# zm0612/funny_lidar_slam

Hardware: NVIDIA H100
Metric: scans/sec (higher is better)
Workload: dtype f64

## Files before the change

### funny_lidar_slam_b200/csrc/fls_api.cu

```cuda
#include <algorithm>
#include <cmath>
#include <cstdlib>
#include <cstring>
#include <new>
#include <vector>

#include "fls_frontend.h"
#include "fls_gn.cuh"
#include "fls_handle.h"

namespace fls {

static thread_local std::string g_last_error;
void set_last_error(const std::string& s) { g_last_error = s; }
const char* last_error_cstr() { return g_last_error.c_str(); }

Handle::Handle(const fls_config& c) : cfg(c) {
    try {
        init();
    } catch (...) {
        release();
        throw;
    }
}
// ... 117 lines not shown
        st->h2d_bytes = h2d_bytes;
        st->d2h_bytes = d2h_bytes;
    }
}

void Handle::set_fit_cloud(const float4* d, size_t n) {
    fit_cloud.reserve(n);
    if (n) FLS_CUDA(cudaMemcpyAsync(fit_cloud.p, d, n * sizeof(float4), cudaMemcpyDeviceToDevice, stream));
    set_fit_view(fit_cloud.p, n);
}

void Handle::set_fit_view(const float4* d, size_t n) {
    fit_pts = d;
    fit_cloud_n = n;
    fit_cloud_version++;
}

GnParams Handle::gn_params(int method, int min_effective) const {
    GnParams p;
    p.method = method;
    p.max_iterations = cfg.max_iterations;
    p.min_effective = min_effective;
    p.rot_thres = cfg.rotation_converge_thres;
    p.pos_thres = cfg.position_converge_thres;
    return p;
}

unsigned Handle::next_ll_epoch(size_t n_records) {
    const size_t cap0 = ll_rows.cap;
    ll_rows.reserve(n_records);
    if (ll_rows.cap != cap0) FLS_CUDA(cudaMemsetAsync(ll_rows.p, 0, ll_rows.cap * sizeof(uint4), stream));
    match_epoch = (match_epoch + 1) & 0xffffffu;
    if (match_epoch == 0) match_epoch = 1;
    return match_epoch << 8;
}

unsigned char* Handle::batch_table(size_t bytes) {
    if (bytes > h_batch_cap) {
        if (h_batch) cudaFreeHost(h_batch);
        h_batch = nullptr;
        h_batch_cap = 0;
        FLS_CUDA(cudaMallocHost(&h_batch, bytes * 2));
        h_batch_cap = bytes * 2;
    }
    d_batch.reserve(bytes);
    return h_batch;
}

void Handle::send_batch_table(size_t bytes) {
    FLS_CUDA(cudaMemcpyAsync(d_batch.p, h_batch, bytes, cudaMemcpyHostToDevice, stream));
    h2d_bytes += (long long)bytes;
}

void Handle::read_back(int B) {
    log_n.assign(1, 0);
    FLS_CUDA(cudaMemcpyAsync(h_state, state.p, sizeof(GnState) * (size_t)B, cudaMemcpyDeviceToHost, stream));
    d2h_bytes += (long long)(sizeof(GnState) * (size_t)B);
    if (log_cap) {
        const size_t bytes = sizeof(fls_iter_log) * (size_t)log_cap * (size_t)B;
        FLS_CUDA(cudaMemcpyAsync(h_log.data(), log.p, bytes, cudaMemcpyDeviceToHost, stream));
        d2h_bytes += (long long)bytes;
    }
}

void Handle::unpack(int B, const size_t* n, double* T, int* converged, fls_match_stats* st) {
    float kernel_ms = 0.f;
    if (profile) FLS_CUDA(cudaEventElapsedTime(&kernel_ms, prof_ev[0], prof_ev[1]));
    for (int s = 0; s < B; ++s) {
        const GnState& gs = h_state[s];
        double* Ts = T + 16 * s;
        for (int r = 0; r < 3; ++r) {
            for (int c = 0; c < 3; ++c) Ts[c * 4 + r] = gs.R[r * 3 + c];
            Ts[12 + r] = gs.t[r];
        }
        Ts[3] = Ts[7] = Ts[11] = 0.0;
        Ts[15] = 1.0;
        if (converged) converged[s] = gs.converged;
        if (st) {
            fls_match_stats& o = st[s];
            if (s > 0) std::memset(&o, 0, sizeof(o));
            o.iterations = gs.iter;
            o.converged = gs.converged;
            o.n_source = (long long)n[s];
            o.n_valid = gs.n_valid;
            o.sum_residual = gs.sum_res;
            if (profile) {
                o.algo_bytes = (long long)gs.iter * (long long)n[s] * per_point_iter_bytes + (long long)(gs.cand_total + 0.5) * per_cand_bytes;
                o.kernel_ms = s == 0 ? kernel_ms : 0.f;
                o.kernel_launches = s == 0 ? 1 : 0;
            }
        }
    }
    std::memcpy(T_final, T, sizeof(T_final));
    log_n.resize(B);
    for (int s = 0; s < B; ++s) log_n[s] = h_state[s].iter < log_cap ? h_state[s].iter : log_cap;
}

static GnLoopCtl make_ctl(Handle& h, int method, int grid, int min_effective) {
    GnLoopCtl c;
    c.tag_base = h.next_ll_epoch((size_t)grid * 32 + kLlPoseLen);
    c.state = h.state.p;
    c.ll_rows = h.ll_rows.p;
    c.ll_pose = h.ll_rows.p + (size_t)grid * 32;
    c.gp = h.gn_params(method, min_effective);
    c.log = h.scan_log(0);
    c.log_cap = h.log_cap;
    c.result = h.scan_result(0);
    return c;
}

static void finish_match(Handle& h, double* T, int* converged, fls_match_stats* st, size_t n_source) {
    h.read_back(1);
    h.end_call(st);
    h.unpack(1, &n_source, T, converged, st);
}

int Handle::add_cloud_ivox(const void* pts, size_t n, size_t stride) {
    if (cfg.localization_mode) ivox.clear();
    else if (ivox.n_pts != 0) return FLS_ERR_UNSUPPORTED;
    const float4* d = upload(pts, n, stride, stage);
    const int rc = ivox.append_and_build(d, n, cfg.ivox_capacity, stream);
    launches += ivox.launches;
    ivox.launches = 0;
    if (cfg.localization_mode) set_fit_cloud(d, n);
    return rc;
}

int Handle::match_ivox_batch(int B, const float4* const* d_scans, const size_t* n, double* T, int* converged, fls_match_stats* st) {
    const int rc = enqueue_ivox_batch(B, d_scans, n, T);
    if (rc != FLS_OK) return rc;
    return finish_ivox_batch(T, converged, st);
}

int Handle::enqueue_ivox_batch(int B, const float4* const* d_scans, const size_t* n, const double* T) {
    if (ivox.n_pts == 0) return FLS_ERR_NO_MAP;
    if (B < 1 || B > kMaxBatch) return FLS_ERR_INVALID_ARG;
    int off[kMaxBatch + 1];
    off[0] = 0;
    int grid = 1;
    const bool use_v9 = B > 1;
    for (int s = 0; s < B; ++s) {
        if (n[s] > 0x3fffffffull || (long long)off[s] + (long long)n[s] > 0x7ffffff0ll) return FLS_ERR_INVALID_ARG;
        off[s + 1] = off[s] + (int)n[s];
        const int g = use_v9 ? p2plane_v9_grid((int)n[s], cfg.device) : p2plane_grid((int)n[s], cfg.device);
        if (g > grid) grid = g;
    }
    const int n_total = off[B];
    const size_t nt = (size_t)n_total;
    rec0.reserve(nt + 1);
    rec1.reserve(nt + 1);
    flags.reserve(nt + 1);
    src_f.reserve(nt + 1);
    const unsigned tag_base = next_ll_epoch((size_t)B * grid * 32 + (size_t)B * kLlPoseLen + (size_t)B * 16 * 32);
    const size_t o_pose = 0, o_off = o_pose + sizeof(PoseArg) * kMaxBatch, o_desc = o_off + sizeof(int) * (kMaxBatch + 4),
                 o_ptr = o_desc + sizeof(P2PlaneScan) * kMaxBatch;
    const size_t tbl_bytes = o_ptr + sizeof(void*) * kMaxBatch;
    unsigned char* const tbl = batch_table(tbl_bytes);
    PoseArg* hp = reinterpret_cast<PoseArg*>(tbl + o_pose);
    int* ho = reinterpret_cast<int*>(tbl + o_off);
    P2PlaneScan* hd = reinterpret_cast<P2PlaneScan*>(tbl + o_desc);
    const float4** hq = reinterpret_cast<const float4**>(tbl + o_ptr);
    uint4* pose_base = ll_rows.p + (size_t)B * grid * 32;
    for (int s = 0; s < B; ++s) {
        const double* Ts = T + 16 * s;
        for (int r = 0; r < 3; ++r) {
            for (int c = 0; c < 3; ++c) hp[s].R[r * 3 + c] = Ts[c * 4 + r];
            hp[s].t[r] = Ts[12 + r];
        }
        ho[s] = off[s];
        hq[s] = d_scans[s];
        P2PlaneScan& d = hd[s];
        d.src = src_f.p + off[s];
        d.n = (int)n[s];
        d.tag_base = tag_base;
        d.state = state.p + s;
        d.rec0 = rec0.p + off[s];
        d.rec1 = rec1.p + off[s];
        d.flags = flags.p + off[s];
        d.rows = ll_rows.p + (size_t)s * grid * 32;
        d.ll_pose = pose_base + (size_t)s * kLlPoseLen;
        d.log = scan_log(s);
        d.result = scan_result(s);
        d.grows = pose_base + (size_t)B * kLlPoseLen + (size_t)s * 16 * 32;
    }
    ho[B] = off[B];
    send_batch_table(tbl_bytes);
    const PoseArg* d_poses = reinterpret_cast<const PoseArg*>(d_batch.p + o_pose);
    const int* d_off = reinterpret_cast<const int*>(d_batch.p + o_off);
    const P2PlaneScan* d_desc = reinterpret_cast<const P2PlaneScan*>(d_batch.p + o_desc);
    const float4* const* d_ptrs = reinterpret_cast<const float4* const*>(d_batch.p + o_ptr);
    prepare_queries(d_ptrs, n_total, d_off, B, d_poses, state.p, ivox_view(), flags.p, src_f.p, scratch, stream, &launches);
    P2PlaneLoopArgs a;
    a.map = ivox_view();
    a.plane_thres = cfg.point_to_planar_thres;
    a.gp = gn_params(FLS_P2PLANE_IVOX, 50);
    a.log_cap = log_cap;
    a.scans = d_desc;
    a.n_scans = B;
    a.tickets = nullptr;
    a.ticket_stride = 0;
    a.abort_word = nullptr;
    gn_launch(16 + 16LL * a.map.n_stencil + 32, 16, d_scans[0], n[0], [&] {
        if (use_v9) {
            a.ticket_stride = cfg.max_iterations + 2;
            tickets.reserve((size_t)B * a.ticket_stride + 4);
            FLS_CUDA(cudaMemsetAsync(tickets.p, 0, sizeof(unsigned) * ((size_t)B * a.ticket_stride + 4), stream));
            a.tickets = tickets.p;
            a.abort_word = tickets.p + (size_t)B * a.ticket_stride;
            launch_p2plane_v9(a, grid, stream);
        } else {
            launch_p2plane_loop(a, grid, stream);
        }
    });
    read_back(B);
    *h_abort = 0;
    if (use_v9) FLS_CUDA(cudaMemcpyAsync(h_abort, a.abort_word, sizeof(unsigned), cudaMemcpyDeviceToHost, stream));
    pend_n.assign(n, n + B);
    pend_v9 = use_v9;
    return FLS_OK;
}

int Handle::finish_ivox_batch(double* T, int* converged, fls_match_stats* st) {
    const int B = (int)pend_n.size();
    if (B < 1) return FLS_ERR_INVALID_ARG;
    end_call(st);
    if (pend_v9 && *h_abort) {
        pend_n.clear();
        set_last_error("p2plane_v9_kernel: watchdog — a wait loop gave up after 4 s (hand-over protocol error)");
        return FLS_ERR_CUDA;
    }
    unpack(B, pend_n.data(), T, converged, st);
    pend_n.clear();
    return FLS_OK;
}

int Handle::match_p2plane_ivox(const float4* d_src, size_t n, double* T, int* converged, fls_match_stats* st) {
    const float4* scans[1] = {d_src};
    const size_t ns[1] = {n};
    int conv = 0;
    const int rc = match_ivox_batch(1, scans, ns, T, &conv, st);
    if (rc != FLS_OK) return rc;
    if (converged) *converged = conv;
    const int ni = (int)n;
    if (h_state->converged && !cfg.localization_mode) {
        stage.reserve(n + 1);
        stage2.reserve(n + 1);
        const GnState& s = *h_state;
        const size_t n_add = select_ivox_inserts(ivox_view(), d_src, ni, s.Rprev, s.tprev, s.R, s.t, 0.5 ,
                                                 stage2.p, stage.p, scratch, stream, &launches);
        const int rc2 = ivox.append_and_build(stage.p, n_add, cfg.ivox_capacity, stream);
        launches += ivox.launches;
        ivox.launches = 0;
        FLS_CUDA(cudaStreamSynchronize(stream));
        if (st) st->gpu_launches = launches;
        if (rc2 != FLS_OK) return rc2;
    }
    return FLS_OK;
}

int Handle::add_cloud_ndt(const float4* d_cloud, size_t n) {
    const int rc = ndt.add_cloud(d_cloud, n, cfg.source_cloud_filter_size, ndt_first_scan, stream);
    launches += ndt.launches;
    ndt.launches = 0;
    if (cfg.localization_mode && rc == FLS_OK) {
        const size_t nf = voxel_grid_device(d_cloud, n, cfg.source_cloud_filter_size, ndt.filtered.p, ndt.scratch, stream, &launches);
        set_fit_cloud(ndt.filtered.p, nf);
    }
    ndt_first_scan = cfg.localization_mode != 0;
    return rc;
}

int Handle::match_ndt(const float4* d_in, size_t n_in, double* T, int* converged, fls_match_stats* st) {
    if (ndt.n_vox == 0) return FLS_ERR_NO_MAP;
    src_f.reserve(n_in);
    const size_t n = voxel_grid_device(d_in, n_in, cfg.source_cloud_filter_size, src_f.p, scratch, stream, &launches);
    const int ni = (int)n;
    const int grid = ndt_grid(ni, cfg.device);
    GnLoopCtl ctl = make_ctl(*this, FLS_NDT, grid, cfg.ndt_min_effective_pts);
    double T_in[16];
    std::memcpy(T_in, T, sizeof(T_in));
    launch_gn_init(state.p, T, stream);
    launches++;
    NdtArgs a;
    a.src = src_f.p;
    a.n = ni;
    a.map = ndt.view();
    a.outlier_thres = cfg.ndt_outlier_thres;
    a.state = state.p;
    gn_launch(16 + 16LL * 7, 80, src_f.p, n, [&] { launch_ndt_loop(a, ctl, grid, stream); });
    finish_match(*this, T, converged, st, n);
    if (!h_state->failed && !cfg.localization_mode) {
        stage2.reserve(n);
        launch_transform_f(src_f.p, n, T_in, stage2.p, stream);
        launches++;
        const int rc2 = add_cloud_ndt(stage2.p, n);
        FLS_CUDA(cudaStreamSynchronize(stream));
        if (st) st->gpu_launches = launches;
        if (rc2 != FLS_OK) return rc2;
    }
    return FLS_OK;
}

int Handle::match_ndt_batch(int B, const float4* const* d_scans, const size_t* n_in, double* T, int* converged, fls_match_stats* st) {
    if (ndt.n_vox == 0) return FLS_ERR_NO_MAP;
    if (B < 1 || B > kMaxBatch) return FLS_ERR_INVALID_ARG;
    size_t total_in = 0;
    for (int s = 0; s < B; ++s) total_in += n_in[s];
    src_f.reserve(total_in + 1);
    size_t off[kMaxBatch + 1];
    off[0] = 0;
    for (int s = 0; s < B; ++s) {
        const size_t nf = voxel_grid_device(d_scans[s], n_in[s], cfg.source_cloud_filter_size, src_f.p + off[s], scratch, stream, &launches);
        if (nf > 0x3fffffffull) return FLS_ERR_INVALID_ARG;
        off[s + 1] = off[s] + nf;
    }
    const int cap = ndt_max_grid(cfg.device);
    int need[kMaxBatch], tot_need = 0;
    for (int s = 0; s < B; ++s) {
        need[s] = (int)((off[s + 1] - off[s] + kNdtBlock - 1) / kNdtBlock);
        if (need[s] < 1) need[s] = 1;
        tot_need += need[s];
    }
    if (B > cap) return FLS_ERR_INVALID_ARG;
    int ncta[kMaxBatch], grid = 0;
    for (int s = 0; s < B; ++s) {
        ncta[s] = tot_need <= cap ? need[s] : (int)((long long)need[s] * (cap - B) / tot_need) + 1;
        grid += ncta[s];
    }
    const unsigned tag_base = next_ll_epoch((size_t)grid * 32 + (size_t)B * kLlPoseLen);
    const size_t tbl_bytes = sizeof(NdtBatchItem) * (size_t)B;
    NdtBatchItem* items = reinterpret_cast<NdtBatchItem*>(batch_table(tbl_bytes));
    uint4* pose_base = ll_rows.p + (size_t)grid * 32;
    size_t ns[kMaxBatch];
    int cta0 = 0;
    for (int s = 0; s < B; ++s) {
        launch_gn_init(state.p + s, T + 16 * s, stream);
        launches++;
        ns[s] = off[s + 1] - off[s];
        NdtBatchItem& it = items[s];
        std::memset(&it, 0, sizeof(it));
        it.a.src = src_f.p + off[s];
        it.a.n = (int)ns[s];
        it.a.map = ndt.view();
        it.a.outlier_thres = cfg.ndt_outlier_thres;
        it.a.state = state.p + s;
        it.ctl.state = state.p + s;
        it.ctl.ll_rows = ll_rows.p + (size_t)cta0 * 32;
        it.ctl.ll_pose = pose_base + (size_t)s * kLlPoseLen;
        it.ctl.tag_base = tag_base;
        it.ctl.gp = gn_params(FLS_NDT, cfg.ndt_min_effective_pts);
        it.ctl.log = scan_log(s);
        it.ctl.log_cap = log_cap;
        it.ctl.result = scan_result(s);
        it.cta0 = cta0;
        it.ncta = ncta[s];
        cta0 += ncta[s];
    }
    send_batch_table(tbl_bytes);
    gn_launch(16 + 16LL * 7, 80, src_f.p, ns[0],
// ... 902 lines not shown
```

### funny_lidar_slam_b200/csrc/fls_kernels.h

```cpp
#pragma once
#include "fls_common.cuh"
#include "fls_gn.cuh"
#include "fls_ivox.cuh"
#include "fls_maps.h"

namespace fls {

static constexpr int kP2PlaneBlock = 768;
static constexpr int kNdtBlock = 512;
static constexpr int kIcpBlock = 512;
static constexpr int kLoamBlock = 256;

static constexpr int kMaxBatch = 64;

struct PoseArg {
    double R[9];
    double t[3];
};

struct P2PlaneScan {
    const float4* src;
    int n;
    unsigned tag_base;
    GnState* state;
    float4* rec0;
    float4* rec1;
    unsigned char* flags;
    uint4* rows;
    uint4* ll_pose;
    fls_iter_log* log;
    double* result;
    uint4* grows;
};

struct P2PlaneLoopArgs {
    IvoxView map;
    double plane_thres;
    GnParams gp;
    int log_cap;
    const P2PlaneScan* scans;
    int n_scans;
    unsigned* tickets;
    int ticket_stride;
    unsigned* abort_word;
};
int p2plane_max_grid(int device);
int p2plane_chunks(int n);
int p2plane_grid(int n, int device);
void launch_p2plane_loop(const P2PlaneLoopArgs& a, int grid, cudaStream_t st);
int p2plane_v9_grid(int n_max, int device);
void launch_p2plane_v9(const P2PlaneLoopArgs& a, int grid, cudaStream_t st);
void prepare_queries(const float4* const* d_scan_ptrs, int n_total, const int* d_offsets, int n_scans, const PoseArg* d_poses, GnState* d_states,
                     const IvoxView& map, unsigned char* d_flags, float4* d_sorted, BuildScratch& sc, cudaStream_t st, int* launches);
size_t select_ivox_inserts(const IvoxView& map, const float4* d_src, int n, const double* R_prev, const double* t_prev, const double* R_fin,
                           const double* t_fin, double filter, float4* d_world, float4* d_out, BuildScratch& sc, cudaStream_t st, int* launches);
void launch_ivox_knn_test(const IvoxView& map, const float4* d_q, int n, float4* d_out, int* d_found, cudaStream_t st);

struct NdtArgs {
    const float4* __restrict__ src;
    int n;
    NdtView map;
    double outlier_thres;
    GnState* state;
};
int ndt_grid(int n, int device);
void launch_ndt_loop(const NdtArgs& a, const GnLoopCtl& ctl, int grid, cudaStream_t st);
struct __align__(16) NdtBatchItem {
    NdtArgs a;
    GnLoopCtl ctl;
    int cta0, ncta;
    int pad[2];
};
int ndt_max_grid(int device);
void launch_ndt_batch(const NdtBatchItem* d_items, int n_scans, int grid, cudaStream_t st);

struct IcpArgs {
    const float4* __restrict__ src;
    int n;
    IvoxView map;
    double max_corr;
    GnState* state;
};
int icp_grid_blocks(int n, int device);
void launch_icp_loop(const IcpArgs& a, const GnLoopCtl& ctl, int grid, cudaStream_t st);

struct LoamGrid {
    const float4* __restrict__ pts;
    const HashSlot* __restrict__ tab;
    unsigned mask;
    float inv_cell, cell;
    unsigned n_pts;
};
struct LoamArgs {
    const float4* __restrict__ corner;
    int n_corner;
    const float4* __restrict__ planar;
    int n_planar;
    LoamGrid corner_map, planar_map;
    double plane_thres;
    double search_thres;
    double line_ratio;
    float gate;
    GnState* state;
    double* __restrict__ rec;
    unsigned char* __restrict__ flags;
};
int loam_grid_blocks(int n, int device);
void launch_loam_loop(const LoamArgs& a, const GnLoopCtl& ctl, int grid, cudaStream_t st);

void launch_fitness(const IvoxView& g, const float4* d_src, int n, const double* T_colmajor, float max_range, double* d_out2, cudaStream_t st);

}
```

### funny_lidar_slam_b200/csrc/fls_p2plane.cu

```cuda
#include <cooperative_groups.h>

#include <cub/cub.cuh>

#include "fls_gn.cuh"
#include "fls_ivox.cuh"
#include "fls_kernels.h"
#include "fls_knn.cuh"
#include "fls_plane.cuh"

namespace fls {
namespace {

__device__ __forceinline__ void knn5_stream(const IvoxView& m, float qx, float qy, float qz, Top5& nn, unsigned& n_cand) {
    nn.init();
    n_cand = 0;
    const unsigned long long key = pack_key(ivox_coord(qx, m.inv_res), ivox_coord(qy, m.inv_res), ivox_coord(qz, m.inv_res));
    unsigned start, count;
    if (!table_find(m.ctab, m.cmask, key, start, count)) return;
    n_cand = count;
    const float4* __restrict__ L = m.lists + start;
    const float r2 = m.max_range2;
    {
        const char* pl = reinterpret_cast<const char*>(L);
        const unsigned bytes = count * 16u;
// ... 138 lines not shown
                    else s_stop[v] = val != 0.0;
                }
            }
        }
        __syncthreads();
        bool live[V];
#pragma unroll
        for (int v = 0; v < V; ++v) {
            live[v] = v < nv && !s_stop[v];
            if (v < nv && s_stop[v]) {
                if (threadIdx.x == 0) s_iter[gs[v]] = 255;
                --n_left;
            }
        }
#pragma unroll 1
        for (int v = 0; v < nv; ++v) {
            if (!live[v]) continue;
            const int s = gs[v];
            const P2PlaneScan* __restrict__ sc = a.scans + s;
            const int folder = s % G;
            const int n = sc->n;
            const int n_chunks = (n + 31) >> 5;
            const float4* __restrict__ src = sc->src;
            float4* __restrict__ rec0 = sc->rec0;
            float4* __restrict__ rec1 = sc->rec1;
            unsigned char* __restrict__ flags = sc->flags;
            const int slot = (cta - folder - 1 + G) % G;
            const double* pose = s_pose[v];

            double acc = 0.0;
            for (int chunk = slot * W + warp; chunk < n_chunks; chunk += n_warps) {
                const int i = (chunk << 5) + lane;
                double J[6] = {0, 0, 0, 0, 0, 0}, ad = 0.0, vflag = 0.0;
                unsigned n_cand = 0, n_fb = 0;
                if (i < n) {
                    const float4 sp = src[i];
                    bool use = p2plane_point(a.map, sp, pose, a.plane_thres, J, ad, n_cand, n_fb);
                    if (use) {
                        rec0[i] = make_float4((float)J[0], (float)J[1], (float)J[2], (float)J[3]);
                        rec1[i] = make_float4((float)J[4], (float)J[5], (float)ad, 1.0f);
                        flags[i] = 1;
                    } else if (flags[i]) {
                        const float4 r0 = rec0[i], r1 = rec1[i];
                        J[0] = r0.x; J[1] = r0.y; J[2] = r0.z; J[3] = r0.w; J[4] = r1.x; J[5] = r1.y;
                        ad = r1.z;
                        use = true;
                    } else {
#pragma unroll
                        for (int k = 0; k < 6; ++k) J[k] = 0.0;
                        ad = 0.0;
                    }
                    vflag = use ? 1.0 : 0.0;
                }
                double* rec = s_rec[warp][lane];
#pragma unroll
                for (int k = 0; k < 6; ++k) rec[k] = J[k];
                rec[kRecAd] = ad;
                rec[kRecValid] = vflag;
                rec[kRecCand] = (double)n_cand;
                rec[kRecHits] = (double)n_fb;
                rec[kRecOne] = 1.0;
                __syncwarp();
#pragma unroll 8
                for (int p = 0; p < 32; ++p) acc += s_rec[warp][p][ca] * s_rec[warp][p][cb];
                __syncwarp();
            }
            s_part[v][warp][lane] = acc * sgn;
        }
        __syncthreads();
        if (warp < nv && live[warp]) {
            const P2PlaneScan* __restrict__ sc = a.scans + gs[warp];
            double val = 0;
#pragma unroll
            for (int w = 0; w < W; ++w) val += s_part[warp][w][lane];
            ll_store(sc->rows + (size_t)cta * 32 + lane, val, sc->tag_base | (unsigned)(git[warp] + 1));
        }
#pragma unroll 1
        for (int v = 0; v < nv; ++v) {
            if (!live[v] || cta != gs[v] % G) continue;
            const P2PlaneScan* __restrict__ sc = a.scans + gs[v];
            GnState* const state = sc->state;
            const int it = git[v];
            const unsigned tag = sc->tag_base | (unsigned)(it + 1);
            uint4* const rows = sc->rows;
            GnPre pre;
            if (threadIdx.x == 0) gn_load(state, pre);
            const int nrows = G;
            double sum;
            for (;;) {
                bool ok = true;
                double a0 = 0, a1 = 0, a2 = 0, a3 = 0;
                int r = warp;
                for (; r + 7 * W < nrows; r += 8 * W) {
                    double v0, v1, v2, v3, v4, v5, v6, v7;
                    const bool k0 = ll_load(rows + (size_t)r * 32 + lane, tag, v0);
                    const bool k1 = ll_load(rows + (size_t)(r + W) * 32 + lane, tag, v1);
                    const bool k2 = ll_load(rows + (size_t)(r + 2 * W) * 32 + lane, tag, v2);
                    const bool k3 = ll_load(rows + (size_t)(r + 3 * W) * 32 + lane, tag, v3);
                    const bool k4 = ll_load(rows + (size_t)(r + 4 * W) * 32 + lane, tag, v4);
                    const bool k5 = ll_load(rows + (size_t)(r + 5 * W) * 32 + lane, tag, v5);
                    const bool k6 = ll_load(rows + (size_t)(r + 6 * W) * 32 + lane, tag, v6);
                    const bool k7 = ll_load(rows + (size_t)(r + 7 * W) * 32 + lane, tag, v7);
                    ok = ok && k0 && k1 && k2 && k3 && k4 && k5 && k6 && k7;
                    a0 += v0; a1 += v1; a2 += v2; a3 += v3;
                    a0 += v4; a1 += v5; a2 += v6; a3 += v7;
                }
                for (; r + 3 * W < nrows; r += 4 * W) {
                    double v0, v1, v2, v3;
                    const bool k0 = ll_load(rows + (size_t)r * 32 + lane, tag, v0);
                    const bool k1 = ll_load(rows + (size_t)(r + W) * 32 + lane, tag, v1);
                    const bool k2 = ll_load(rows + (size_t)(r + 2 * W) * 32 + lane, tag, v2);
                    const bool k3 = ll_load(rows + (size_t)(r + 3 * W) * 32 + lane, tag, v3);
                    ok = ok && k0 && k1 && k2 && k3;
                    a0 += v0; a1 += v1; a2 += v2; a3 += v3;
                }
                for (; r < nrows; r += W) {
                    double v0;
                    ok = ok && ll_load(rows + (size_t)r * 32 + lane, tag, v0);
                    a0 += v0;
                }
                sum = (a0 + a1) + (a2 + a3);
                if (__all_sync(0xffffffffu, ok)) break;
                __nanosleep(100);
            }
            s_red[warp][lane] = sum;
            __syncthreads();
            if (warp == 0) {
                double t = 0;
#pragma unroll
                for (int w = 0; w < W; ++w) t += s_red[w][lane];
                __syncwarp();
                s_red[0][lane] = t;
                __syncwarp();
                if (lane == 0) gn_step_pre(state, pre, s_red[0], a.gp, sc->log, a.log_cap, sc->ll_pose, tag, sc->result);
            }
            __syncthreads();
        }
        if (threadIdx.x == 0)
            for (int v = 0; v < nv; ++v)
                if (live[v]) s_iter[gs[v]] = (unsigned char)(git[v] + 1);
        __syncthreads();
    }
}

__device__ __forceinline__ unsigned spread_bits3(unsigned v) {
    v &= 0x3ffu;
    v = (v | (v << 16)) & 0x030000ffu;
    v = (v | (v << 8)) & 0x0300f00fu;
    v = (v | (v << 4)) & 0x030c30c3u;
    v = (v | (v << 2)) & 0x09249249u;
    return v;
}

__global__ void p2plane_prep_kernel(const float4* const* __restrict__ scan_ptrs, int n_total, const int* __restrict__ offsets, int n_scans,
                                    const PoseArg* __restrict__ poses, float inv_res, int hbits, unsigned* __restrict__ keys,
                                    unsigned* __restrict__ idx, unsigned char* __restrict__ flags, GnState* __restrict__ states,
                                    const HashSlot* __restrict__ ctab, unsigned cmask, const float4* __restrict__ lists) {
    const int i = blockIdx.x * blockDim.x + threadIdx.x;
    if (blockIdx.x == 0 && (int)threadIdx.x < n_scans) {
        GnState* s = states + threadIdx.x;
        const PoseArg& pose = poses[threadIdx.x];
        for (int k = 0; k < 9; ++k) s->R[k] = s->R0[k] = s->Rprev[k] = pose.R[k];
        for (int k = 0; k < 3; ++k) s->t[k] = s->t0[k] = s->tprev[k] = pose.t[k];
        s->last_rot = s->last_pos = 0.0;
        s->sum_res = 0;
        s->cand_total = s->hits_total = 0;
        s->n_valid = 0;
        s->iter = 0;
        s->done = 0;
        s->converged = 0;
        s->failed = 0;
    }
    if (i >= n_total) return;
    flags[i] = 0;
    int sid = 0;
    {
        int lo = 0, hi = n_scans;
        while (hi - lo > 1) {
            const int mid = (lo + hi) >> 1;
            if (__ldg(offsets + mid) <= i) lo = mid;
            else hi = mid;
        }
        sid = lo;
    }
    const float4 sp = scan_ptrs[sid][i - __ldg(offsets + sid)];
    const PoseArg& pose = poses[sid];
    const float qx = xform_row_d(__ldg(&pose.R[0]), __ldg(&pose.R[1]), __ldg(&pose.R[2]), __ldg(&pose.t[0]), sp.x, sp.y, sp.z);
    const float qy = xform_row_d(__ldg(&pose.R[3]), __ldg(&pose.R[4]), __ldg(&pose.R[5]), __ldg(&pose.t[1]), sp.x, sp.y, sp.z);
    const float qz = xform_row_d(__ldg(&pose.R[6]), __ldg(&pose.R[7]), __ldg(&pose.R[8]), __ldg(&pose.t[2]), sp.x, sp.y, sp.z);
    const unsigned kx = (unsigned)ivox_coord(qx, inv_res), ky = (unsigned)ivox_coord(qy, inv_res), kz = (unsigned)ivox_coord(qz, inv_res);
    const unsigned lo = spread_bits3(kx & 15u) | (spread_bits3(ky & 15u) << 1) | (spread_bits3(kz & 15u) << 2);
    const unsigned hm = (1u << hbits) - 1u;
    const unsigned hx = (kx >> 4) & hm, hy = (ky >> 4) & hm;
    unsigned hi = 0;
    for (int b = 0; b < hbits; ++b) hi |= (((hx >> b) & 1u) << (2 * b)) | (((hy >> b) & 1u) << (2 * b + 1));
    keys[i] = lo | (hi << 12) | ((unsigned)sid << (12 + 2 * hbits));
    idx[i] = (unsigned)i;
    if (ctab) {
        const unsigned long long key = pack_key((int)kx, (int)ky, (int)kz);
        const unsigned peers = __match_any_sync(__activemask(), key);
        if ((int)(__ffs(peers) - 1) == (int)(threadIdx.x & 31)) {
            unsigned start, count;
            if (table_find(ctab, cmask, key, start, count)) {
                const char* p = reinterpret_cast<const char*>(lists + start);
                const unsigned bytes = count * 16u;
                for (unsigned off = 0; off < bytes; off += 128u) asm volatile("prefetch.global.L2 [%0];" ::"l"(p + off));
                asm volatile("prefetch.global.L2 [%0];" ::"l"(p + bytes - 1));
            }
        }
    }
}

__global__ void gather4_kernel(const float4* const* __restrict__ scan_ptrs, const int* __restrict__ offsets, int n_scans,
                               const unsigned* __restrict__ idx, int n, float4* __restrict__ dst) {
    const int i = blockIdx.x * blockDim.x + threadIdx.x;
    if (i >= n) return;
    const int g = (int)idx[i];
    int lo = 0, hi = n_scans;
    while (hi - lo > 1) {
        const int mid = (lo + hi) >> 1;
        if (__ldg(offsets + mid) <= g) lo = mid;
        else hi = mid;
    }
    dst[i] = scan_ptrs[lo][g - __ldg(offsets + lo)];
}

__global__ void ivox_knn_test_kernel(IvoxView map, const float4* __restrict__ q, int n, float4* __restrict__ out, int* __restrict__ found) {
    const int i = blockIdx.x * blockDim.x + threadIdx.x;
    if (i >= n) return;
    const float4 p = q[i];
    Top5 nn;
    unsigned nc;
    knn5_stream(map, p.x, p.y, p.z, nn, nc);
    const unsigned js[5] = {nn.idx(nn.k0), nn.idx(nn.k1), nn.idx(nn.k2), nn.idx(nn.k3), nn.idx(nn.k4)};
    int f = 0;
    for (int k = 0; k < 5; ++k) {
        if (js[k] != 0xffffffffu) {
            out[(size_t)i * 5 + k] = map.lists[js[k]];
            ++f;
        } else {
            out[(size_t)i * 5 + k] = make_float4(0, 0, 0, 0);
        }
    }
    found[i] = f;
}

__global__ void ivox_insert_rule_kernel(IvoxView map, const float4* __restrict__ src, int n, PoseArg prev, PoseArg fin, double filter,
                                        unsigned char* __restrict__ cls, float4* __restrict__ world) {
    const int i = blockIdx.x * blockDim.x + threadIdx.x;
    if (i >= n) return;
    const float4 sp = src[i];
    const float qx = xform_row_d(prev.R[0], prev.R[1], prev.R[2], prev.t[0], (double)sp.x, (double)sp.y, (double)sp.z);
    const float qy = xform_row_d(prev.R[3], prev.R[4], prev.R[5], prev.t[1], (double)sp.x, (double)sp.y, (double)sp.z);
    const float qz = xform_row_d(prev.R[6], prev.R[7], prev.R[8], prev.t[2], (double)sp.x, (double)sp.y, (double)sp.z);
    Top5 nn;
    unsigned nc;
    knn5_stream(map, qx, qy, qz, nn, nc);
    const float wx = xform_row_d(fin.R[0], fin.R[1], fin.R[2], fin.t[0], (double)sp.x, (double)sp.y, (double)sp.z);
    const float wy = xform_row_d(fin.R[3], fin.R[4], fin.R[5], fin.t[1], (double)sp.x, (double)sp.y, (double)sp.z);
    const float wz = xform_row_d(fin.R[6], fin.R[7], fin.R[8], fin.t[2], (double)sp.x, (double)sp.y, (double)sp.z);
    world[i] = make_float4(wx, wy, wz, sp.w);
    const unsigned js[5] = {nn.k0, nn.k1, nn.k2, nn.k3, nn.k4};
    if (js[0] == 0xffffffffu) {
        cls[i] = 1;
        return;
    }
    const double pv[3] = {(double)wx, (double)wy, (double)wz};
    double c[3];
#pragma unroll
    for (int a = 0; a < 3; ++a) c[a] = (floor(pv[a] / filter) + 0.5) * filter;
    const float4 n0 = __ldg(map.lists + js[0]);
    const double half = 0.5 * filter;
    if (fabs((double)n0.x - c[0]) > half && fabs((double)n0.y - c[1]) > half && fabs((double)n0.z - c[2]) > half) {
        cls[i] = 2;
        return;
    }
    bool need = true;
    const double dist = (pv[0] - c[0]) * (pv[0] - c[0]) + (pv[1] - c[1]) * (pv[1] - c[1]) + (pv[2] - c[2]) * (pv[2] - c[2]);
    if (js[4] != 0xffffffffu) {
#pragma unroll
        for (int r = 0; r < 5; ++r) {
            const float4 m = __ldg(map.lists + js[r]);
            const double ex = (double)m.x - c[0], ey = (double)m.y - c[1], ez = (double)m.z - c[2];
            if (ex * ex + ey * ey + ez * ez < dist + 1.0e-6) need = false;
        }
    }
    cls[i] = need ? 1 : 0;
}

__global__ void ivox_insert_keys_kernel(const unsigned char* __restrict__ cls, int n, unsigned long long* __restrict__ ones) {
    const int i = blockIdx.x * blockDim.x + threadIdx.x;
    if (i < n) ones[i] = (cls[i] == 1 ? 1ull : 0ull) | (cls[i] == 2 ? (1ull << 32) : 0ull);
}
__global__ void ivox_insert_scatter_kernel(const unsigned char* __restrict__ cls, const unsigned long long* __restrict__ excl, int n,
                                           const float4* __restrict__ world, float4* __restrict__ out, unsigned long long* __restrict__ total) {
    const int i = blockIdx.x * blockDim.x + threadIdx.x;
    if (i >= n) return;
    const unsigned long long last = excl[n - 1] + ((cls[n - 1] == 1 ? 1ull : 0ull) | (cls[n - 1] == 2 ? (1ull << 32) : 0ull));
    const unsigned n1 = (unsigned)(last & 0xffffffffull);
    if (i == 0) *total = last;
    const unsigned char c = cls[i];
    if (c == 1) out[(unsigned)(excl[i] & 0xffffffffull)] = world[i];
    else if (c == 2) out[n1 + (unsigned)(excl[i] >> 32)] = world[i];
}

constexpr int kMinB = 1;
const void* p2plane_fn() { return (const void*)p2plane_gn_kernel<kP2PlaneBlock, kMinB>; }
size_t p2plane_smem() {
    constexpr int W = kP2PlaneBlock / 32, V = kVisitGroup < W ? kVisitGroup : W;
    return (size_t)W * 32 * kRecW * sizeof(double) + (size_t)V * W * 32 * sizeof(double);
}

}

int p2plane_max_grid(int device) {
    static int cached[64] = {0};
    if (device >= 0 && device < 64 && cached[device]) return cached[device];
    int sms = 0;
    cudaDeviceGetAttribute(&sms, cudaDevAttrMultiProcessorCount, device);
    int per_sm = 0;
    cudaFuncSetAttribute(p2plane_fn(), cudaFuncAttributeMaxDynamicSharedMemorySize, (int)p2plane_smem());
    cudaOccupancyMaxActiveBlocksPerMultiprocessor(&per_sm, p2plane_gn_kernel<kP2PlaneBlock, kMinB>, kP2PlaneBlock, p2plane_smem());
    const int g = sms * (per_sm > 0 ? per_sm : 1);
    if (device >= 0 && device < 64) cached[device] = g;
    return g;
}

int p2plane_chunks(int n) { return (n + 31) / 32; }

int p2plane_grid(int n, int device) {
    const int W = kP2PlaneBlock / 32;
    const int need = (p2plane_chunks(n) + W - 1) / W;
    const int cap = p2plane_max_grid(device);
    const int g = need + 1 < cap ? need + 1 : cap;
    return g > 0 ? g : 1;
}

void launch_p2plane_loop(const P2PlaneLoopArgs& a, int grid, cudaStream_t st) {
    P2PlaneLoopArgs args = a;
    void* params[] = {&args};
    FLS_CUDA(cudaLaunchCooperativeKernel(p2plane_fn(), dim3(grid), dim3(kP2PlaneBlock), params, p2plane_smem(), st));
}

void prepare_queries(const float4* const* d_scan_ptrs, int n_total, const int* d_offsets, int n_scans, const PoseArg* d_poses, GnState* d_states,
                     const IvoxView& map, unsigned char* d_flags, float4* d_sorted, BuildScratch& sc, cudaStream_t st, int* launches) {
    const int m = n_total > 0 ? n_total : 1;
    sc.k32a.reserve(m);
    sc.k32b.reserve(m);
    sc.idx.reserve(m);
    sc.idx_sorted.reserve(m);
    constexpr int key_bits = 16;
    int scan_bits = 0;
    while ((1 << scan_bits) < n_scans) ++scan_bits;
    p2plane_prep_kernel<<<(m + 255) / 256, 256, 0, st>>>(d_scan_ptrs, n_total, d_offsets, n_scans, d_poses, map.inv_res, (key_bits - 12) / 2, sc.k32a.p,
                                                        sc.idx.p, d_flags, d_states, map.ctab, map.cmask, map.lists);
    if (launches) *launches += 1;
    if (n_total <= 0) return;
    const int sort_bits = key_bits + scan_bits;
    size_t t1 = 0;
    cub::DeviceRadixSort::SortPairs(nullptr, t1, sc.k32a.p, sc.k32b.p, sc.idx.p, sc.idx_sorted.p, n_total, 0, sort_bits, st);
    sc.cub_tmp.reserve(t1 + 256);
    size_t tb = sc.cub_tmp.cap;
    FLS_CUDA(cub::DeviceRadixSort::SortPairs(sc.cub_tmp.p, tb, sc.k32a.p, sc.k32b.p, sc.idx.p, sc.idx_sorted.p, n_total, 0, sort_bits, st));
    gather4_kernel<<<(n_total + 255) / 256, 256, 0, st>>>(d_scan_ptrs, d_offsets, n_scans, sc.idx_sorted.p, n_total, d_sorted);
    if (launches) *launches += 2 + (sort_bits + 7) / 8 + 1;
}

size_t select_ivox_inserts(const IvoxView& map, const float4* d_src, int n, const double* R_prev, const double* t_prev, const double* R_fin,
                           const double* t_fin, double filter, float4* d_world, float4* d_out, BuildScratch& sc, cudaStream_t st, int* launches) {
    if (n <= 0) return 0;
    PoseArg prev, fin;
    for (int k = 0; k < 9; ++k) {
        prev.R[k] = R_prev[k];
        fin.R[k] = R_fin[k];
    }
    for (int k = 0; k < 3; ++k) {
        prev.t[k] = t_prev[k];
        fin.t[k] = t_fin[k];
    }
    sc.minmax.reserve((size_t)n / 4 + 16);
    unsigned char* cls = reinterpret_cast<unsigned char*>(sc.minmax.p);
    sc.keys.reserve((size_t)n + 1);
    sc.keys_sorted.reserve((size_t)n + 1);
    const int g = (n + 127) / 128;
    ivox_insert_rule_kernel<<<g, 128, 0, st>>>(map, d_src, n, prev, fin, filter, cls, d_world);
    ivox_insert_keys_kernel<<<(n + 255) / 256, 256, 0, st>>>(cls, n, sc.keys.p);
    size_t tb = 0;
    cub::DeviceScan::ExclusiveSum(nullptr, tb, sc.keys.p, sc.keys_sorted.p, n, st);
    sc.cub_tmp.reserve(tb + 256);
    tb = sc.cub_tmp.cap;
    FLS_CUDA(cub::DeviceScan::ExclusiveSum(sc.cub_tmp.p, tb, sc.keys.p, sc.keys_sorted.p, n, st));
    unsigned long long* d_total = sc.keys.p + n;
    ivox_insert_scatter_kernel<<<(n + 255) / 256, 256, 0, st>>>(cls, sc.keys_sorted.p, n, d_world, d_out, d_total);
    unsigned long long total = 0;
    FLS_CUDA(cudaMemcpyAsync(&total, d_total, sizeof(total), cudaMemcpyDeviceToHost, st));
    FLS_CUDA(cudaStreamSynchronize(st));
    if (launches) *launches += 4;
    return (size_t)(total & 0xffffffffull) + (size_t)(total >> 32);
}

void launch_ivox_knn_test(const IvoxView& map, const float4* d_q, int n, float4* d_out, int* d_found, cudaStream_t st) {
    if (n <= 0) return;
    ivox_knn_test_kernel<<<(n + 127) / 128, 128, 0, st>>>(map, d_q, n, d_out, d_found);
}

}
```

Measured before the change: 10240.

## Replace global radix sort with per-tile block sort fused into prep kernel

Query preparation used to run a prep kernel, a multi-pass CUB device radix sort and a gather kernel. It now does the key computation, a per-tile cub::BlockRadixSort over 8192-point tiles and the gather in one kernel. The ticket memset also moves into that kernel. This removes several launches and the global sort passes. In exchange, spatial ordering is only local within each tile, which could weaken locality in the later Gauss-Newton loop.

```diff
diff --git a/funny_lidar_slam_b200/csrc/fls_api.cu b/funny_lidar_slam_b200/csrc/fls_api.cu
--- a/funny_lidar_slam_b200/csrc/fls_api.cu
+++ b/funny_lidar_slam_b200/csrc/fls_api.cu
@@ -293,12 +293,14 @@
     flags.reserve(nt + 1);
     src_f.reserve(nt + 1);
     const unsigned tag_base = next_ll_epoch((size_t)B * grid * 32 + (size_t)B * kLlPoseLen + (size_t)B * 16 * 32);
-    const size_t o_pose = 0, o_off = o_pose + sizeof(PoseArg) * kMaxBatch, o_desc = o_off + sizeof(int) * (kMaxBatch + 4),
-                 o_ptr = o_desc + sizeof(P2PlaneScan) * kMaxBatch;
+    const size_t o_pose = 0, o_off = o_pose + sizeof(PoseArg) * kMaxBatch, o_toff = o_off + sizeof(int) * (kMaxBatch + 4),
+                 o_desc = o_toff + sizeof(int) * (kMaxBatch + 4), o_ptr = o_desc + sizeof(P2PlaneScan) * kMaxBatch;
     const size_t tbl_bytes = o_ptr + sizeof(void*) * kMaxBatch;
     unsigned char* const tbl = batch_table(tbl_bytes);
     PoseArg* hp = reinterpret_cast<PoseArg*>(tbl + o_pose);
     int* ho = reinterpret_cast<int*>(tbl + o_off);
+    int* ht = reinterpret_cast<int*>(tbl + o_toff);
+    ht[0] = 0;
     P2PlaneScan* hd = reinterpret_cast<P2PlaneScan*>(tbl + o_desc);
     const float4** hq = reinterpret_cast<const float4**>(tbl + o_ptr);
     uint4* pose_base = ll_rows.p + (size_t)B * grid * 32;
@@ -309,6 +311,7 @@
             hp[s].t[r] = Ts[12 + r];
         }
         ho[s] = off[s];
+        ht[s + 1] = ht[s] + order_tiles((int)n[s]);
         hq[s] = d_scans[s];
         P2PlaneScan& d = hd[s];
         d.src = src_f.p + off[s];
@@ -328,9 +331,14 @@
     send_batch_table(tbl_bytes);
     const PoseArg* d_poses = reinterpret_cast<const PoseArg*>(d_batch.p + o_pose);
     const int* d_off = reinterpret_cast<const int*>(d_batch.p + o_off);
+    const int* d_toff = reinterpret_cast<const int*>(d_batch.p + o_toff);
     const P2PlaneScan* d_desc = reinterpret_cast<const P2PlaneScan*>(d_batch.p + o_desc);
     const float4* const* d_ptrs = reinterpret_cast<const float4* const*>(d_batch.p + o_ptr);
-    prepare_queries(d_ptrs, n_total, d_off, B, d_poses, state.p, ivox_view(), flags.p, src_f.p, scratch, stream, &launches);
+    const int ticket_stride = cfg.max_iterations + 2;
+    const int n_tickets = use_v9 ? B * ticket_stride + 4 : 0;
+    if (use_v9) tickets.reserve((size_t)n_tickets);
+    prepare_queries(d_ptrs, d_off, d_toff, ht[B], B, d_poses, state.p, ivox_view(), flags.p, src_f.p, use_v9 ? tickets.p : nullptr, n_tickets,
+                    stream, &launches);
     P2PlaneLoopArgs a;
     a.map = ivox_view();
     a.plane_thres = cfg.point_to_planar_thres;
@@ -343,9 +351,7 @@
     a.abort_word = nullptr;
     gn_launch(16 + 16LL * a.map.n_stencil + 32, 16, d_scans[0], n[0], [&] {
         if (use_v9) {
-            a.ticket_stride = cfg.max_iterations + 2;
-            tickets.reserve((size_t)B * a.ticket_stride + 4);
-            FLS_CUDA(cudaMemsetAsync(tickets.p, 0, sizeof(unsigned) * ((size_t)B * a.ticket_stride + 4), stream));
+            a.ticket_stride = ticket_stride;
             a.tickets = tickets.p;
             a.abort_word = tickets.p + (size_t)B * a.ticket_stride;
             launch_p2plane_v9(a, grid, stream);
diff --git a/funny_lidar_slam_b200/csrc/fls_kernels.h b/funny_lidar_slam_b200/csrc/fls_kernels.h
--- a/funny_lidar_slam_b200/csrc/fls_kernels.h
+++ b/funny_lidar_slam_b200/csrc/fls_kernels.h
@@ -50,8 +50,11 @@
 void launch_p2plane_loop(const P2PlaneLoopArgs& a, int grid, cudaStream_t st);
 int p2plane_v9_grid(int n_max, int device);
 void launch_p2plane_v9(const P2PlaneLoopArgs& a, int grid, cudaStream_t st);
-void prepare_queries(const float4* const* d_scan_ptrs, int n_total, const int* d_offsets, int n_scans, const PoseArg* d_poses, GnState* d_states,
-                     const IvoxView& map, unsigned char* d_flags, float4* d_sorted, BuildScratch& sc, cudaStream_t st, int* launches);
+static constexpr int kOrderTile = 8192;
+inline int order_tiles(int n) { return (n + kOrderTile - 1) / kOrderTile; }
+void prepare_queries(const float4* const* d_scan_ptrs, const int* d_offsets, const int* d_tile_off, int n_tiles, int n_scans,
+                     const PoseArg* d_poses, GnState* d_states, const IvoxView& map, unsigned char* d_flags, float4* d_sorted,
+                     unsigned* d_zero, int n_zero, cudaStream_t st, int* launches);
 size_t select_ivox_inserts(const IvoxView& map, const float4* d_src, int n, const double* R_prev, const double* t_prev, const double* R_fin,
                            const double* t_fin, double filter, float4* d_world, float4* d_out, BuildScratch& sc, cudaStream_t st, int* launches);
 void launch_ivox_knn_test(const IvoxView& map, const float4* d_q, int n, float4* d_out, int* d_found, cudaStream_t st);
diff --git a/funny_lidar_slam_b200/csrc/fls_p2plane.cu b/funny_lidar_slam_b200/csrc/fls_p2plane.cu
--- a/funny_lidar_slam_b200/csrc/fls_p2plane.cu
+++ b/funny_lidar_slam_b200/csrc/fls_p2plane.cu
@@ -314,77 +314,86 @@
     return v;
 }
 
-__global__ void p2plane_prep_kernel(const float4* const* __restrict__ scan_ptrs, int n_total, const int* __restrict__ offsets, int n_scans,
-                                    const PoseArg* __restrict__ poses, float inv_res, int hbits, unsigned* __restrict__ keys,
-                                    unsigned* __restrict__ idx, unsigned char* __restrict__ flags, GnState* __restrict__ states,
-                                    const HashSlot* __restrict__ ctab, unsigned cmask, const float4* __restrict__ lists) {
-    const int i = blockIdx.x * blockDim.x + threadIdx.x;
-    if (blockIdx.x == 0 && (int)threadIdx.x < n_scans) {
-        GnState* s = states + threadIdx.x;
-        const PoseArg& pose = poses[threadIdx.x];
-        for (int k = 0; k < 9; ++k) s->R[k] = s->R0[k] = s->Rprev[k] = pose.R[k];
-        for (int k = 0; k < 3; ++k) s->t[k] = s->t0[k] = s->tprev[k] = pose.t[k];
-        s->last_rot = s->last_pos = 0.0;
-        s->sum_res = 0;
-        s->cand_total = s->hits_total = 0;
-        s->n_valid = 0;
-        s->iter = 0;
-        s->done = 0;
-        s->converged = 0;
-        s->failed = 0;
-    }
-    if (i >= n_total) return;
-    flags[i] = 0;
+constexpr int kOrdThreads = 512, kOrdItems = kOrderTile / kOrdThreads;
+
+__global__ void __launch_bounds__(kOrdThreads) p2plane_prep_kernel(const float4* const* __restrict__ scan_ptrs, const int* __restrict__ offsets,
+                                                                   const int* __restrict__ tile_off, int n_scans, const PoseArg* __restrict__ poses,
+                                                                   float inv_res, unsigned* __restrict__ zero, int n_zero,
+                                                                   unsigned char* __restrict__ flags, GnState* __restrict__ states,
+                                                                   float4* __restrict__ dst, const HashSlot* __restrict__ ctab, unsigned cmask,
+                                                                   const float4* __restrict__ lists) {
+    using Sort = cub::BlockRadixSort<unsigned, kOrdThreads, kOrdItems, unsigned>;
+    __shared__ typename Sort::TempStorage s_sort;
+    if (blockIdx.x == 0) {
+        if ((int)threadIdx.x < n_scans) {
+            GnState* s = states + threadIdx.x;
+            const PoseArg& pose = poses[threadIdx.x];
+            for (int k = 0; k < 9; ++k) s->R[k] = s->R0[k] = s->Rprev[k] = pose.R[k];
+            for (int k = 0; k < 3; ++k) s->t[k] = s->t0[k] = s->tprev[k] = pose.t[k];
+            s->last_rot = s->last_pos = 0.0;
+            s->sum_res = 0;
+            s->cand_total = s->hits_total = 0;
+            s->n_valid = 0;
+            s->iter = 0;
+            s->done = 0;
+            s->converged = 0;
+            s->failed = 0;
+        }
+        for (int k = threadIdx.x; k < n_zero; k += blockDim.x) zero[k] = 0;
+    }
+    const int tile = (int)blockIdx.x;
+    if (tile >= __ldg(tile_off + n_scans)) return;
     int sid = 0;
     {
         int lo = 0, hi = n_scans;
         while (hi - lo > 1) {
             const int mid = (lo + hi) >> 1;
-            if (__ldg(offsets + mid) <= i) lo = mid;
+            if (__ldg(tile_off + mid) <= tile) lo = mid;
             else hi = mid;
         }
         sid = lo;
     }
-    const float4 sp = scan_ptrs[sid][i - __ldg(offsets + sid)];
+    const int first = __ldg(offsets + sid) + (tile - __ldg(tile_off + sid)) * kOrderTile;
+    const int n_here = min(kOrderTile, __ldg(offsets + sid + 1) - first);
+    const float4* __restrict__ src = scan_ptrs[sid] + (first - __ldg(offsets + sid));
     const PoseArg& pose = poses[sid];
-    const float qx = xform_row_d(__ldg(&pose.R[0]), __ldg(&pose.R[1]), __ldg(&pose.R[2]), __ldg(&pose.t[0]), sp.x, sp.y, sp.z);
-    const float qy = xform_row_d(__ldg(&pose.R[3]), __ldg(&pose.R[4]), __ldg(&pose.R[5]), __ldg(&pose.t[1]), sp.x, sp.y, sp.z);
-    const float qz = xform_row_d(__ldg(&pose.R[6]), __ldg(&pose.R[7]), __ldg(&pose.R[8]), __ldg(&pose.t[2]), sp.x, sp.y, sp.z);
-    const unsigned kx = (unsigned)ivox_coord(qx, inv_res), ky = (unsigned)ivox_coord(qy, inv_res), kz = (unsigned)ivox_coord(qz, inv_res);
-    const unsigned lo = spread_bits3(kx & 15u) | (spread_bits3(ky & 15u) << 1) | (spread_bits3(kz & 15u) << 2);
-    const unsigned hm = (1u << hbits) - 1u;
-    const unsigned hx = (kx >> 4) & hm, hy = (ky >> 4) & hm;
-    unsigned hi = 0;
-    for (int b = 0; b < hbits; ++b) hi |= (((hx >> b) & 1u) << (2 * b)) | (((hy >> b) & 1u) << (2 * b + 1));
-    keys[i] = lo | (hi << 12) | ((unsigned)sid << (12 + 2 * hbits));
-    idx[i] = (unsigned)i;
-    if (ctab) {
-        const unsigned long long key = pack_key((int)kx, (int)ky, (int)kz);
-        const unsigned peers = __match_any_sync(__activemask(), key);
-        if ((int)(__ffs(peers) - 1) == (int)(threadIdx.x & 31)) {
-            unsigned start, count;
-            if (table_find(ctab, cmask, key, start, count)) {
-                const char* p = reinterpret_cast<const char*>(lists + start);
-                const unsigned bytes = count * 16u;
-                for (unsigned off = 0; off < bytes; off += 128u) asm volatile("prefetch.global.L2 [%0];" ::"l"(p + off));
-                asm volatile("prefetch.global.L2 [%0];" ::"l"(p + bytes - 1));
+    unsigned key[kOrdItems], pos[kOrdItems];
+#pragma unroll
+    for (int k = 0; k < kOrdItems; ++k) {
+        const int q = k * kOrdThreads + (int)threadIdx.x;
+        pos[k] = (unsigned)q;
+        key[k] = 1u << 16;
+        if (q < n_here) {
+            flags[first + q] = 0;
+            const float4 sp = src[q];
+            const float qx = xform_row_d(__ldg(&pose.R[0]), __ldg(&pose.R[1]), __ldg(&pose.R[2]), __ldg(&pose.t[0]), sp.x, sp.y, sp.z);
+            const float qy = xform_row_d(__ldg(&pose.R[3]), __ldg(&pose.R[4]), __ldg(&pose.R[5]), __ldg(&pose.t[1]), sp.x, sp.y, sp.z);
+            const float qz = xform_row_d(__ldg(&pose.R[6]), __ldg(&pose.R[7]), __ldg(&pose.R[8]), __ldg(&pose.t[2]), sp.x, sp.y, sp.z);
+            const unsigned kx = (unsigned)ivox_coord(qx, inv_res), ky = (unsigned)ivox_coord(qy, inv_res), kz = (unsigned)ivox_coord(qz, inv_res);
+            const unsigned lo = spread_bits3(kx & 15u) | (spread_bits3(ky & 15u) << 1) | (spread_bits3(kz & 15u) << 2);
+            const unsigned hx = (kx >> 4) & 3u, hy = (ky >> 4) & 3u;
+            key[k] = lo | (((hx & 1u) | ((hy & 1u) << 1) | ((hx & 2u) << 1) | ((hy & 2u) << 2)) << 12);
+            if (ctab) {
+                const unsigned long long vkey = pack_key((int)kx, (int)ky, (int)kz);
+                const unsigned peers = __match_any_sync(__activemask(), vkey);
+                if ((int)(__ffs(peers) - 1) == (int)(threadIdx.x & 31)) {
+                    unsigned start, count;
+                    if (table_find(ctab, cmask, vkey, start, count)) {
+                        const char* p = reinterpret_cast<const char*>(lists + start);
+                        const unsigned bytes = count * 16u;
+                        for (unsigned off = 0; off < bytes; off += 128u) asm volatile("prefetch.global.L2 [%0];" ::"l"(p + off));
+                        asm volatile("prefetch.global.L2 [%0];" ::"l"(p + bytes - 1));
+                    }
+                }
             }
         }
     }
-}
-
-__global__ void gather4_kernel(const float4* const* __restrict__ scan_ptrs, const int* __restrict__ offsets, int n_scans,
-                               const unsigned* __restrict__ idx, int n, float4* __restrict__ dst) {
-    const int i = blockIdx.x * blockDim.x + threadIdx.x;
-    if (i >= n) return;
-    const int g = (int)idx[i];
-    int lo = 0, hi = n_scans;
-    while (hi - lo > 1) {
-        const int mid = (lo + hi) >> 1;
-        if (__ldg(offsets + mid) <= g) lo = mid;
-        else hi = mid;
-    }
-    dst[i] = scan_ptrs[lo][g - __ldg(offsets + lo)];
+    Sort(s_sort).SortBlockedToStriped(key, pos, 0, 17);
+#pragma unroll
+    for (int k = 0; k < kOrdItems; ++k) {
+        const int r = k * kOrdThreads + (int)threadIdx.x;
+        if (r < n_here) dst[first + r] = src[pos[k]];
+    }
 }
 
 __global__ void ivox_knn_test_kernel(IvoxView map, const float4* __restrict__ q, int n, float4* __restrict__ out, int* __restrict__ found) {
@@ -504,28 +513,12 @@
     FLS_CUDA(cudaLaunchCooperativeKernel(p2plane_fn(), dim3(grid), dim3(kP2PlaneBlock), params, p2plane_smem(), st));
 }
 
-void prepare_queries(const float4* const* d_scan_ptrs, int n_total, const int* d_offsets, int n_scans, const PoseArg* d_poses, GnState* d_states,
-                     const IvoxView& map, unsigned char* d_flags, float4* d_sorted, BuildScratch& sc, cudaStream_t st, int* launches) {
-    const int m = n_total > 0 ? n_total : 1;
-    sc.k32a.reserve(m);
-    sc.k32b.reserve(m);
-    sc.idx.reserve(m);
-    sc.idx_sorted.reserve(m);
-    constexpr int key_bits = 16;
-    int scan_bits = 0;
-    while ((1 << scan_bits) < n_scans) ++scan_bits;
-    p2plane_prep_kernel<<<(m + 255) / 256, 256, 0, st>>>(d_scan_ptrs, n_total, d_offsets, n_scans, d_poses, map.inv_res, (key_bits - 12) / 2, sc.k32a.p,
-                                                        sc.idx.p, d_flags, d_states, map.ctab, map.cmask, map.lists);
+void prepare_queries(const float4* const* d_scan_ptrs, const int* d_offsets, const int* d_tile_off, int n_tiles, int n_scans,
+                     const PoseArg* d_poses, GnState* d_states, const IvoxView& map, unsigned char* d_flags, float4* d_sorted,
+                     unsigned* d_zero, int n_zero, cudaStream_t st, int* launches) {
+    p2plane_prep_kernel<<<n_tiles > 0 ? n_tiles : 1, kOrdThreads, 0, st>>>(d_scan_ptrs, d_offsets, d_tile_off, n_scans, d_poses, map.inv_res, d_zero,
+                                                                          n_zero, d_flags, d_states, d_sorted, map.ctab, map.cmask, map.lists);
     if (launches) *launches += 1;
-    if (n_total <= 0) return;
-    const int sort_bits = key_bits + scan_bits;
-    size_t t1 = 0;
-    cub::DeviceRadixSort::SortPairs(nullptr, t1, sc.k32a.p, sc.k32b.p, sc.idx.p, sc.idx_sorted.p, n_total, 0, sort_bits, st);
-    sc.cub_tmp.reserve(t1 + 256);
-    size_t tb = sc.cub_tmp.cap;
-    FLS_CUDA(cub::DeviceRadixSort::SortPairs(sc.cub_tmp.p, tb, sc.k32a.p, sc.k32b.p, sc.idx.p, sc.idx_sorted.p, n_total, 0, sort_bits, st));
-    gather4_kernel<<<(n_total + 255) / 256, 256, 0, st>>>(d_scan_ptrs, d_offsets, n_scans, sc.idx_sorted.p, n_total, d_sorted);
-    if (launches) *launches += 2 + (sort_bits + 7) / 8 + 1;
 }
 
 size_t select_ivox_inserts(const IvoxView& map, const float4* d_src, int n, const double* R_prev, const double* t_prev, const double* R_fin,
```

After: 11040, median of 6. +7.8%, better.
